# NicolaDM/MAPLE

Measured on AMD Instinct MI355X. Metric: candidate SPR placements/sec, higher is better.
Workload: dtype f64

## Files before the change

include/maple_hip_debug.h:

```cpp
#ifndef MAPLE_HIP_DEBUG_H
#define MAPLE_HIP_DEBUG_H
#include "maple_hip.h"

#ifdef __cplusplus
extern "C" {
#endif

int maple_debug_frontier_levels(maple_ctx *ctx, int32_t cap, int64_t *itemsUpdating, int64_t *itemsCached, float *msUpdating,
                                float *msCached, int32_t *n, int64_t *waveItemsSmall , int64_t *waveItemsBig );

int maple_debug_wave_append_batch(maple_ctx *ctx, int32_t n, const int32_t *parentList, const int32_t *childList,
                                  const uint8_t *isTipC, const double *bLen, double *outLK, float *ms);
int maple_debug_trace_query(maple_ctx *ctx, int32_t query);
int maple_debug_calib_walk(maple_ctx *ctx, uint64_t bytes, int32_t repeats, float *ms);
int maple_debug_calib_write(maple_ctx *ctx, uint64_t bytes, int32_t mode, int32_t repeats, float *ms);
int maple_debug_trace_read(maple_ctx *ctx, int32_t *n, int32_t *items4 , double *vals2 );
int maple_debug_gpv_batch(maple_ctx *ctx, int32_t n, const int32_t *i12, const double *totLen, const double *M16,
                          const double *errorRate, const double *vect4, const uint8_t *upNode, const uint8_t *flag,
                          double *out4);
int maple_debug_simplify_batch(maple_ctx *ctx, int32_t n, const double *vec4, const int32_t *refA, int32_t *out);
int maple_debug_frontier_pass_batch(maple_ctx *ctx, int32_t n, const int32_t *list, const int32_t *mutList, const uint8_t *dirIsUp,
                                    int32_t waveForm, int32_t *outList, uint8_t *grade, uint8_t *sameHandle);

#ifdef __cplusplus
}
#endif
#endif
```

maple_amd/csrc/batch_host.h:

```cpp
#pragma once
#include "ctx_host.h"

#include <algorithm>
#include <cstring>
#include <vector>

struct alignas(16) TileBest { double score; int32_t rank, idx; };

#ifndef MAPLE_BLOCK
#define MAPLE_BLOCK 256
#endif
#ifndef MAPLE_APPEND_WAVES
#define MAPLE_APPEND_WAVES 4
#endif
#define MAPLE_APPEND_ATTR __launch_bounds__(MAPLE_BLOCK) __attribute__((amdgpu_waves_per_eu(MAPLE_APPEND_WAVES, MAPLE_APPEND_WAVES)))
#ifndef MAPLE_ZERO_DIST_BUDGET
#define MAPLE_ZERO_DIST_BUDGET 16
#endif

static int grid_for(int n)
{
    int g = (n + MAPLE_BLOCK - 1) / MAPLE_BLOCK;
    if (g < 1) g = 1;
    if (g > 256 * 8) g = 256 * 8;
// ... 13 lines not shown
static inline int ev_pair(maple_ctx *c, hipEvent_t *a, hipEvent_t *b, int kind = 0, double units = 0.0, double bytes = 0.0)
{
    return maple_internal_ev_pair(c, a, b, kind, units, bytes);
}

template <class T> static int h2d(maple_ctx *c, DevBuf<T> &b, const T *src, size_t n)
{
    HIPCK(c, b.reserve(n ? n : 1));
    if (n) HIPCK(c, hipMemcpyAsync(b.p, src, n * sizeof(T), hipMemcpyHostToDevice, c->stream));
    return MAPLE_OK;
}

static int stage_begin(maple_ctx *c, size_t bytes)
{
    c->stg_cur ^= 1;
    const int k = c->stg_cur;
    bytes += 4096;
    if (bytes > c->stg_cap[k]) {
        HIPCK(c, hipStreamSynchronize(c->stream));
        if (c->stg_h[k]) (void)hipHostFree(c->stg_h[k]);
        if (c->stg_d[k]) (void)hipFree(c->stg_d[k]);
        c->stg_h[k] = nullptr; c->stg_d[k] = nullptr; c->stg_cap[k] = 0;
        const size_t want = std::max(bytes * 2, (size_t)1 << 20);
        HIPCK(c, hipHostMalloc((void **)&c->stg_h[k], want, hipHostMallocDefault));
        HIPCK(c, hipMalloc((void **)&c->stg_d[k], want));
        c->stg_cap[k] = want;
    }
    c->stg_used = c->stg_flushed = 0;
    return MAPLE_OK;
}
template <class T> static T *stage_put(maple_ctx *c, const T *src, size_t n)
{
    const int k = c->stg_cur;
    const size_t off = (c->stg_used + 15) & ~(size_t)15, bytes = n * sizeof(T);
    if (off + bytes > c->stg_cap[k]) return nullptr;
    if (bytes) memcpy(c->stg_h[k] + off, src, bytes);
    c->stg_used = off + bytes;
    return (T *)(c->stg_d[k] + off);
}
static int stage_flush(maple_ctx *c)
{
    const int k = c->stg_cur;
    if (c->stg_used > c->stg_flushed)
        HIPCK(c, hipMemcpyAsync(c->stg_d[k] + c->stg_flushed, c->stg_h[k] + c->stg_flushed, c->stg_used - c->stg_flushed,
                                hipMemcpyHostToDevice, c->stream));
    c->stg_flushed = c->stg_used;
    return MAPLE_OK;
}
#define STAGE(var, c, src, n) auto *var = stage_put((c), (src), (size_t)(n)); if (!var) return fail((c), MAPLE_ERR_NOMEM, "argument staging overflow")

static int need_model(maple_ctx *c)
{
    if (!c->model_set) return fail(c, MAPLE_ERR_STATE, "maple_set_model has not been called");
    return MAPLE_OK;
}


__attribute__((visibility("hidden")))
int commit_lists(maple_ctx *c, int32_t n, const int64_t *d_woff, const int64_t *d_aoff, int32_t *d_n_ent, int32_t *d_n_aux,
                 int32_t *outList, const uint2 *srcW = nullptr, const double *srcA = nullptr);
__attribute__((visibility("hidden")))
int commit_known(maple_ctx *c, int32_t n, const int64_t *d_woff, const int64_t *d_aoff, const int32_t *d_n_ent, const int32_t *d_n_aux,
                 const std::vector<int32_t> &ne, const std::vector<int32_t> &na, int32_t *outList, const uint2 *srcW, const double *srcA);
__attribute__((visibility("hidden")))
int settle(maple_ctx *c);
__attribute__((visibility("hidden")))
int evaluate_placement_items(maple_ctx *c, int32_t n, const int32_t *midTot, const int32_t *down, const int32_t *up, const double *dist,
                             const int32_t *rem, const uint8_t *remTip, const uint8_t *fromTip1, double *out4, double *comp2);
__attribute__((visibility("hidden")))
void launch_wave_append(maple_ctx *c, int grid, int n, const int32_t *pl, const int32_t *cl, const uint8_t *tip, const double *bl, double *out);
__attribute__((visibility("hidden")))
int launch_append_queries(maple_ctx *c, hipStream_t s, int nQ, const int32_t *qList, int nC, const int32_t *cand, int isTip, double bLen,
                          double *out, long long ldOut, const int32_t *outCol, const uint8_t *qTip, const double *qBLen, int kind,
                          double algBytes, TileBest *tileBest = nullptr, const int32_t *visitRank = nullptr, const int4 *chunkTab = nullptr,
                          int nChunkTab = 0, int nF = 1, unsigned long long *finMask = nullptr, bool lanesOnly = false);
__attribute__((visibility("hidden")))
int launch_place_score(maple_ctx *c, int nQ, int nF, const int32_t *qFrameLists, int nC, const int32_t *cand, const int32_t *candFrame,
                       int isTip, double bLen, double *out, long long ldOut, const int32_t *outCol, const uint8_t *qTip, const double *qBLen,
                       int kind = MAPLE_K_PLACE_SCORE, double algBytes = 0.0);
__attribute__((visibility("hidden")))
void update_scratch_free(maple_ctx *c);
__attribute__((visibility("hidden")))
int tree_rebuild_from_host(maple_ctx *c);
```

maple_amd/csrc/debug_abi.hip:

```cpp
#include "../../include/maple_hip_debug.h"
#include "genome_dev.h"
#include "ctx_host.h"
#include "batch_host.h"
#include "frontier.h"
#include "frontier_dev.h"

#include <algorithm>

using namespace frt;

__global__ __launch_bounds__(MAPLE_BLOCK) void k_calib_walk(const unsigned long long *buf, long long nLists, unsigned long long *sink)
{
    unsigned long long acc = 0;
    for (long long l = (long long)blockIdx.x * blockDim.x + threadIdx.x; l < nLists; l += (long long)gridDim.x * blockDim.x) {
        const unsigned long long *p = buf + l * 64;
        unsigned idx = 0;
        for (int k = 0; k < 64; k++) {
            unsigned long long w = p[idx];
            acc += w;
            idx = (idx + 1 + (unsigned)(w & 0)) & 63;
        }
    }
    if (acc == 0x123456789abcdefull) *sink = acc;
}
// ... 210 lines not shown
                                                              int32_t *nAux, uint8_t *grade)
{
    for (int i = blockIdx.x * blockDim.x + threadIdx.x; i < n; i += gridDim.x * blockDim.x) {
        const int h = handle[i];
        if (h >= 0 && h < fp.capL) {
            const LRec r = fp.trec[h];
            woff[i] = LREC_OFF(r.x); aoff[i] = LREC_OFF(r.y); nEnt[i] = LREC_N(r.x); nAux[i] = LREC_N(r.y); grade[i] = fp.tflag[h];
        } else { woff[i] = 0; aoff[i] = 0; nEnt[i] = -1; nAux[i] = 0; grade[i] = 0; }
    }
}

extern "C" int maple_debug_frontier_pass_batch(maple_ctx *c, int32_t n, const int32_t *list, const int32_t *mutList, const uint8_t *dirIsUp,
                                               int32_t waveForm, int32_t *outList, uint8_t *grade, uint8_t *sameHandle)
{
    if (!c || n < 0 || n > (1 << 20) || !list || !mutList || !dirIsUp || !outList || !grade || !sameHandle) return MAPLE_ERR_ARG;
    if (n == 0) return MAPLE_OK;
    HIPCK(c, hipSetDevice(c->device));
    TRY(need_model(c));
    TRY(check_ids(c, n, list, false, "list"));
    TRY(settle(c));
    const int32_t nml = (int32_t)c->h_mut_cnt.size();
    long long capW = 0, capA = 0;
    int capE = 1;
    for (int i = 0; i < n; i++) {
        if (mutList[i] < -1 || mutList[i] >= nml) return fail(c, MAPLE_ERR_ARG, "mutList[%d] = %d is not a mutation-list id", i, mutList[i]);
        const long long cnt = mutList[i] < 0 ? 0 : c->h_mut_cnt[mutList[i]];
        const long long ne = c->h_n_ent[list[i]] + 2 * cnt, na = c->h_n_aux[list[i]] + 4 * cnt;
        capW += ne; capA += na;
        capE = std::max(capE, (int)ne);
    }
    const int threads = waveForm ? 64 * std::min(n, 1024) : std::min(1024, (n + FR_BLOCK - 1) / FR_BLOCK * FR_BLOCK);
    const int grid = (threads + FR_BLOCK - 1) / FR_BLOCK;
    const long long lanes = (long long)grid * FR_BLOCK;
    HIPCK(c, c->s_words.reserve((size_t)capW));
    HIPCK(c, c->s_aux.reserve((size_t)capA));
    auto up16 = [](size_t x) { return (x + 255) & ~(size_t)255; };
    const size_t oRec = 0, oCtr = up16(oRec + (size_t)n * sizeof(LRec)), oSw = up16(oCtr + sizeof(FCtr)),
                 oSa = up16(oSw + (waveForm ? 0 : (size_t)lanes * capE * sizeof(uint2))),
                 oWoff = up16(oSa + (waveForm ? 0 : (size_t)lanes * 5 * capE * sizeof(double))), oAoff = up16(oWoff + (size_t)n * 8),
                 oHandle = up16(oAoff + (size_t)n * 8), oNe = up16(oHandle + (size_t)n * 4), oNa = up16(oNe + (size_t)n * 4),
                 oFlag = up16(oNa + (size_t)n * 4), oGrade = up16(oFlag + (size_t)n), total = up16(oGrade + (size_t)n);
    uint8_t *buf = nullptr;
    HIPCK(c, hipMalloc((void **)&buf, total));
    int rc = MAPLE_OK;
    std::vector<int32_t> handle(n);
    do {
        if (hipMemsetAsync(buf, 0, oSw, c->stream) != hipSuccess) { rc = fail(c, MAPLE_ERR_HIP, "hipMemsetAsync"); break; }
        FPools fp;
        memset(&fp, 0, sizeof fp);
        fp.tw = c->s_words.p; fp.ta = c->s_aux.p;
        fp.trec = (LRec *)(buf + oRec); fp.tflag = buf + oFlag;
        fp.capW = capW; fp.capA = capA; fp.capL = n;
        fp.sw = (uint2 *)(buf + oSw); fp.sa = (double *)(buf + oSa); fp.capE = capE;
        fp.ctr = (FCtr *)(buf + oCtr);
        fp.mat = 1;
        fp.mv = MutViewS{c->d_mut3, c->d_mut_off, c->d_mut_cnt};
        const ArenaViewS av{c->d_words, c->d_aux, c->d_ent_off, c->d_aux_off, c->d_n_ent, c->d_n_aux};
        if ((rc = stage_begin(c, (size_t)n * 64 + 256)) != MAPLE_OK) break;
        auto *dl = stage_put(c, list, (size_t)n);
        auto *dml = stage_put(c, mutList, (size_t)n);
        auto *dup = stage_put(c, dirIsUp, (size_t)n);
        if (!dl || !dml || !dup) { rc = fail(c, MAPLE_ERR_NOMEM, "argument staging overflow"); break; }
        if ((rc = stage_flush(c)) != MAPLE_OK) break;
        int32_t *dHandle = (int32_t *)(buf + oHandle), *dNe = (int32_t *)(buf + oNe), *dNa = (int32_t *)(buf + oNa);
        int64_t *dWoff = (int64_t *)(buf + oWoff), *dAoff = (int64_t *)(buf + oAoff);
        if (waveForm) DISPATCH3(c, k_debug_fpass_wave, <<<grid, FR_BLOCK, 0, c->stream>>>(c->d_model, av, fp, n, dl, dml, dup, dHandle));
        else DISPATCH3(c, k_debug_fpass_lane, <<<grid, FR_BLOCK, 0, c->stream>>>(c->d_model, av, fp, n, dl, dml, dup, dHandle));
        hipLaunchKernelGGL(k_debug_fpass_out, dim3(grid_for(n)), dim3(FR_BLOCK), 0, c->stream, fp, n, dHandle, dWoff, dAoff, dNe, dNa, buf + oGrade);
        if (hipGetLastError() != hipSuccess || hipMemcpyAsync(handle.data(), dHandle, (size_t)n * 4, hipMemcpyDeviceToHost, c->stream) != hipSuccess
            || hipMemcpyAsync(grade, buf + oGrade, (size_t)n, hipMemcpyDeviceToHost, c->stream) != hipSuccess
            || hipStreamSynchronize(c->stream) != hipSuccess) { rc = fail(c, MAPLE_ERR_HIP, "the frontier pass hook's launch failed"); break; }
        for (int i = 0; i < n && rc == MAPLE_OK; i++) {
            sameHandle[i] = handle[i] == -(list[i] + 10);
            if (!sameHandle[i] && handle[i] < 0) rc = fail(c, MAPLE_ERR_NOMEM, "item %d: no room for the new list (%d)", i, handle[i]);
        }
        if (rc != MAPLE_OK) break;
        if ((rc = commit_lists(c, n, dWoff, dAoff, dNe, dNa, outList, fp.tw, fp.ta)) != MAPLE_OK) break;
        if (hipStreamSynchronize(c->stream) != hipSuccess) { rc = fail(c, MAPLE_ERR_HIP, "hipStreamSynchronize"); break; }
        for (int i = 0; i < n; i++) if (sameHandle[i]) outList[i] = list[i];
    } while (0);
    (void)hipFree(buf);
    return rc;
}
```

maple_amd/csrc/spr_batch.hip:

```cpp
#include "../../include/maple_hip.h"
#include "genome_dev.h"
#include "search_dev.h"
#include "placement_dev.h"
#include "append_lds.h"
#include "wave_dev.h"
#include "wave_update.h"

#include <algorithm>
#include <chrono>
#include <cfloat>
#include <cmath>
#include <cstdarg>
#include <cstdio>
#include <cstring>
#include <functional>
#include <string>
#include <vector>

using namespace maple;

#include <hipcub/hipcub.hpp>
#include "ctx_host.h"
#include "batch_host.h"
#include "frontier.h"
// ... 837 lines not shown

    const int32_t nT = c->dtree.n;
    std::vector<int32_t> byRank(nT, -1);
    for (int i = 0; i < nT; i++) byRank[c->h_nodes[i].preRank] = i;
    std::vector<SScan> sc((size_t)nT);
    std::vector<int32_t> size(nT, 1), depth(nT, 0);
    std::vector<uint8_t> reach(nT, 0);
    int32_t maxDepth = 0;
    if (!c->tree_stale && c->place && (int)c->h_depth.size() == nT && !c->place->order.empty() && c->place->order[0] == c->dtree.root) {
        for (const int32_t v : c->place->order) { reach[v] = 1; depth[v] = c->h_depth[v]; maxDepth = std::max(maxDepth, depth[v]); }
    } else {
        std::vector<int32_t> stk{c->dtree.root};
        while (!stk.empty()) {
            const int v = stk.back();
            stk.pop_back();
            reach[v] = 1;
            if (c->h_tree_c0[v] >= 0) { stk.push_back(c->h_tree_c0[v]); stk.push_back(c->h_tree_c1[v]); }
        }
        for (int r = 0; r < nT; r++) {
            const int v = byRank[r];
            const int u = c->h_tree_up[v];
            if (reach[v] && u >= 0 && v != c->dtree.root && c->h_nodes[u].preRank < r) depth[v] = depth[u] + 1;
            maxDepth = std::max(maxDepth, depth[v]);
        }
    }
    for (int r = nT - 1; r >= 0; r--) {
        const int v = byRank[r];
        const int u = c->h_tree_up[v];
        if (reach[v] && u >= 0 && v != c->dtree.root && c->h_nodes[u].preRank < r) size[u] += size[v];
    }
    for (int r = 0; r < nT; r++) {
        const int v = byRank[r];
        const NodeRec &nr = c->h_nodes[v];
        uint32_t fl = 0;
        if (nr.up >= 0 && (nr.dist > P.effNon0 || nr.upIsRoot)) fl |= SS_SCORED;
        if (nr.totUp >= 0) fl |= SS_TOTUP;
        if (nr.c0 >= 0) fl |= SS_INNER;
        if (nr.up >= 0 && (nr.whichChild ? c->h_nodes[nr.up].upLeft : c->h_nodes[nr.up].upRight) >= 0) fl |= SS_ENTER;
        sc[r] = SScan{v, size[v], depth[v], ((uint32_t)nr.frameOf << 4) | fl};
    }
    std::vector<int32_t> prank((size_t)nT, 0);
    for (int r = 0; r < nT; r++) { const int u = c->h_tree_up[byRank[r]]; prank[r] = u >= 0 ? c->h_nodes[u].preRank : 0; }
    std::vector<int32_t> candBefore((size_t)nT + 1, 0), cladeVisits((size_t)nT, 0);
    for (int r = 0; r < nT; r++)
        candBefore[r + 1] = candBefore[r] + ((sc[r].ff & SS_TOTUP) ? 1 : 0);
    for (int r = nT - 1; r >= 1; r--) {
        const int v = byRank[r];
        if (!reach[v]) continue;
        const uint32_t fl = sc[r].ff & 15u;
        if (!(fl & SS_ENTER)) continue;
        const bool scored = fl & SS_SCORED, counts = scored && (fl & SS_TOTUP), dropped = scored && !(fl & SS_TOTUP);
        const int add = (counts ? 1 : 0) + ((!dropped && (fl & SS_INNER)) ? cladeVisits[r] : 0);
        cladeVisits[prank[r]] += add;
    }
    TRY(h2d(c, c->t_cand_before, candBefore.data(), candBefore.size()));
    TRY(h2d(c, c->t_clade_visits, cladeVisits.data(), cladeVisits.size()));
    TRY(h2d(c, c->t_scan, sc.data(), sc.size()));
    TRY(h2d(c, c->t_scan_parent, prank.data(), prank.size()));
    HIPCK(c, hipStreamSynchronize(c->stream));
    c->tree_max_depth = maxDepth;
    c->scan_eff = P.effNon0;
    c->scan_valid = true;
    return MAPLE_OK;
}

__global__ __launch_bounds__(64) void k_finite_prefix(int nRows, int nWords, const unsigned long long *mask, int32_t *prefix)
{
    const int lane = threadIdx.x;
    for (int row = blockIdx.x; row < nRows; row += gridDim.x) {
        const unsigned long long *m = mask + (size_t)row * nWords;
        int32_t *p = prefix + (size_t)row * (nWords + 1);
        int run = 0;
        for (int base = 0; base <= nWords; base += 64) {
            const int w = base + lane;
            const int cnt = w < nWords ? __popcll(m[w]) : 0;
            int incl = cnt;
            for (int off = 1; off < 64; off <<= 1) { const int t = __shfl_up(incl, off, 64); if (lane >= off) incl += t; }
            if (w <= nWords) p[w] = run + incl - cnt;
            run += __shfl(incl, 63, 64);
        }
    }
}

static int lists_to_root_frame(maple_ctx *c, std::vector<int32_t> &ids, std::vector<int32_t> fr)
{
    const PlaceMeta &Fm = *c->place;
    std::vector<int32_t> who, src, ml, out;
    std::vector<uint8_t> dir;
    for (;;) {
        who.clear(); src.clear(); ml.clear();
        for (size_t k = 0; k < ids.size(); k++)
            if (fr[k] != 0 && ids[k] >= 0) { who.push_back((int32_t)k); src.push_back(ids[k]); ml.push_back(c->h_tree_mut[Fm.frameNode[fr[k]]]); }
        if (who.empty()) return MAPLE_OK;
        dir.assign(who.size(), 1);
        out.resize(who.size());
        TRY(maple_pass_branch_batch(c, (int32_t)who.size(), src.data(), ml.data(), dir.data(), out.data()));
        for (size_t i = 0; i < who.size(); i++) { ids[who[i]] = out[i]; fr[who[i]] = Fm.frameParent[fr[who[i]]]; }
    }
}
static int ensure_cand_root(maple_ctx *c)
{
    if (c->cand_root_end >= 0) return MAPLE_OK;
    if (c->cand_root_mark >= 0 && c->cand_root_top == (int64_t)c->h_n_ent.size())
        TRY(maple_arena_release(c, c->cand_root_mark | ((int64_t)c->h_mut_cnt.size() << 40)));
    c->cand_root_mark = c->cand_root_top = -1;
    const int64_t begin = (int64_t)c->h_n_ent.size();
    std::vector<int32_t> candRoot(c->h_cand_ids);
    TRY(lists_to_root_frame(c, candRoot, c->h_cand_frame));
    TRY(h2d(c, c->s_cand_root, candRoot.data(), candRoot.size()));
    HIPCK(c, hipStreamSynchronize(c->stream));
    c->cand_root_end = (int64_t)c->h_n_ent.size();
    c->cand_root_mark = begin; c->cand_root_top = c->cand_root_end;
    return MAPLE_OK;
}

extern "C" int maple_spr_search_batch(maple_ctx *c, int32_t n, const int32_t *nodes, const maple_search_params *sp,
                                      int32_t ws_entries_per_lane, int32_t *bestNode, double *bestScore, double *blen3,
                                      int32_t *placement, double *improvement, double *currentLK, int32_t *nAppend,
                                      int32_t *status, int32_t *outRprList)
{
    if (!c || n < 0 || !nodes || !sp || !bestNode || !bestScore || !blen3 || !placement || !improvement || !currentLK
        || !nAppend || !status)
        return MAPLE_ERR_ARG;
    if (n == 0) return MAPLE_OK;
    HIPCK(c, hipSetDevice(c->device));
    TRY(need_model(c));
    if (!c->tree_set) return fail(c, MAPLE_ERR_STATE, "maple_tree_upload has not been called");
    for (int i = 0; i < n; i++)
        if (nodes[i] < 0 || nodes[i] >= c->dtree.n) return fail(c, MAPLE_ERR_ARG, "nodes[%d] = %d is not a node", i, nodes[i]);
    bool patchedOnly = false;
    c->last_search_frontier_only = false;
    if (c->tree_stale) {
        patchedOnly = c->nodes_current && !c->tree_has_mut && n <= 64 && sp->searchTier == 0 && c->trace_query < 0 && !outRprList;
        for (int i = 0; i < n && patchedOnly; i++)
            if (sp->wideSearchBudget >= 0 && !c->dm.usingErrorRate && c->h_tree_dist[nodes[i]] == 0.0) patchedOnly = false;
        if (!patchedOnly) TRY(tree_rebuild_from_host(c));
    }
    const bool dbgT = c->tuning.verbose != 0;
    auto tnow = [] { return std::chrono::steady_clock::now(); };
    auto tms = [](std::chrono::steady_clock::time_point a, std::chrono::steady_clock::time_point b) {
        return std::chrono::duration_cast<std::chrono::microseconds>(b - a).count() * 1e-3;
    };
    const auto tStart = tnow();
    SearchParams P;
    P.strict = sp->strictTopologyStopRules; P.allowedFails = sp->allowedFailsTopology;
    P.thrLKtopology = sp->thresholdLogLKtopology; P.thrPlacement = sp->thresholdTopologyPlacement;
    P.thrOptTopo = sp->thresholdLogLKoptimizationTopology; P.thrConsec = sp->thresholdLogLKconsecutivePlacement;
    P.effNon0 = sp->effectivelyNon0BLen;
    HIPCK(c, c->s_search_out.reserve((size_t)n * sizeof(SearchOut)));
    HIPCK(c, c->s_counter.reserve(8));
    std::vector<SearchOut> &ho = c->h_search_out;
    ho.assign((size_t)n, SearchOut{});
    std::vector<uint8_t> hintedNow;
    std::vector<int32_t> todo(nodes, nodes + n), slot(n);
    for (int i = 0; i < n; i++) slot[i] = i;
    long long poolCapW = 0, poolCapA = 0;
    uint2 *poolW = nullptr;
    double *poolA = nullptr;
    if (outRprList) {
        for (int i = 0; i < n; i++) {
            int lid = c->h_tree_lower[nodes[i]];
            long long ne = lid >= 0 ? c->h_n_ent[lid] : 0, na = lid >= 0 ? c->h_n_aux[lid] : 0;
            poolCapW += 3 * ne + 64; poolCapA += 3 * na + 5 * ne + 64;
        }
        HIPCK(c, c->s_pool_w.reserve((size_t)poolCapW));
        HIPCK(c, c->s_pool_a.reserve((size_t)poolCapA));
        poolW = c->s_pool_w.p; poolA = c->s_pool_a.p;
    }
    HIPCK(c, hipMemsetAsync(c->s_counter.p, 0, 8 * sizeof(int32_t), c->stream));
    unsigned long long *poolUsed = (unsigned long long *)(c->s_counter.p + 2);
    if (dbgT) fprintf(stderr, "[maple] t=%.1f ms: result records cleared\n", tms(tStart, tnow()));
    const int capW0 = ws_entries_per_lane > 0 ? ws_entries_per_lane : std::max(16384, 64 * c->tree_max_ent);
    bool heavyQueries = false;
    bool assistOK = !c->dm.usingErrorRate;
    const bool assistFew = !c->dm.usingErrorRate;
    const bool useFrontier = sp->searchTier == 0 && c->trace_query < 0;
    const std::vector<int32_t> *rowOverride = nullptr;
    FiniteRows finRows{nullptr, nullptr, 0};
    const int finWords = (c->n_scored + 63) / 64;
    auto fin_reserve = [&](size_t rows) -> int {
        HIPCK(c, c->s_fin_mask.reserve_exact(std::max(rows * (size_t)finWords, c->s_fin_mask.cap)));
        HIPCK(c, c->s_fin_prefix.reserve_exact(std::max(rows * (size_t)(finWords + 1), c->s_fin_prefix.cap)));
// ... 175 lines not shown
    std::vector<int32_t> preIdx, preRowOf;
    int preSpare = 0;
    const int nTpre = c->dtree.n;
    const bool matPre = c->tree_has_mut;
    int64_t preMark = -1;
    std::vector<int32_t> preFrameParent, preFrameNode;
    auto pre_rows_max = [&]() -> size_t {
        size_t freeB = 0, totalB = 0;
        size_t budgetB = (size_t)4ull << 30;
        if (hipMemGetInfo(&freeB, &totalB) == hipSuccess)
            budgetB = std::max(budgetB, std::min((freeB + c->s_cache.cap * sizeof(double)) / 2, (size_t)96ull << 30));
        return budgetB / ((size_t)nTpre * sizeof(double));
    };
    auto pre_rows = [&](const bool witnessOK) -> int {
        const size_t rowsMax = pre_rows_max();
        if (preIdx.size() < 64 || preIdx.size() > rowsMax) preIdx.clear();
        else {
            preSpare = witnessOK ? (int)std::min<size_t>(4096, rowsMax - preIdx.size()) : 0;
            const int mZ = (int)preIdx.size();
            HIPCK(c, c->s_cache.reserve_exact((size_t)(mZ + preSpare) * nTpre));
            TRY(fin_reserve((size_t)mZ + preSpare));
            if (!c->stream2) {
                HIPCK(c, hipStreamCreateWithFlags(&c->stream2, hipStreamNonBlocking));
                HIPCK(c, hipEventCreateWithFlags(&c->ev_fork, hipEventDisableTiming));
                HIPCK(c, hipEventCreateWithFlags(&c->ev_join, hipEventDisableTiming));
            }
            std::vector<int32_t> ql(mZ);
            std::vector<uint8_t> qt(mZ);
            std::vector<double> qb(mZ);
            preRowOf.assign(n, -1);
            double qBytes = 0.0;
            for (int k = 0; k < mZ; k++) {
                const int node = nodes[preIdx[k]];
                ql[k] = c->h_tree_lower[node]; qt[k] = c->h_tree_tip[node]; qb[k] = c->h_tree_dist[node];
                preRowOf[preIdx[k]] = k;
                qBytes += 8.0 * c->h_n_ent[ql[k]] + 8.0 * c->h_n_aux[ql[k]];
                if (witnessOK && qb[k] != 0.0) return fail(c, MAPLE_ERR_FATAL, "a search with removedBLen %g among the searches of the witness filter", qb[k]);
            }
            if (matPre) {
                const PlaceMeta &Fm = *c->place;
                TRY(ensure_cand_root(c));
                TRY(maple_arena_mark(c, &preMark));
                std::vector<int32_t> qf(mZ);
                for (int k = 0; k < mZ; k++) qf[k] = Fm.frameOf[nodes[preIdx[k]]];
                TRY(lists_to_root_frame(c, ql, qf));
                if (dbgT) fprintf(stderr, "[maple] t=%.1f ms: their removed lists in the root's frame\n", tms(tStart, tnow()));
                preFrameParent = Fm.frameParent;
                preFrameNode = Fm.frameNode;
                useFin = true;
            }
            HIPCK(c, c->z_ql.reserve(mZ)); HIPCK(c, c->z_qt.reserve(mZ)); HIPCK(c, c->z_qb.reserve(mZ));
            HIPCK(c, hipEventRecord(c->ev_fork, c->stream));
            HIPCK(c, hipStreamWaitEvent(c->stream2, c->ev_fork, 0));
            HIPCK(c, hipMemcpyAsync(c->z_ql.p, ql.data(), (size_t)mZ * sizeof(int32_t), hipMemcpyHostToDevice, c->stream2));
            HIPCK(c, hipMemcpyAsync(c->z_qt.p, qt.data(), (size_t)mZ, hipMemcpyHostToDevice, c->stream2));
            HIPCK(c, hipMemcpyAsync(c->z_qb.p, qb.data(), (size_t)mZ * sizeof(double), hipMemcpyHostToDevice, c->stream2));
            HIPCK(c, hipStreamSynchronize(c->stream2));
            afterLaunch = [c, mZ, nTpre, qBytes, fin_prefix, useFin, finWords, dbgT, matPre, witnessOK]() -> int {
                if (witnessOK && useFin && !c->tuning.denseWideScoring) {
                    long long pairs = 0;
                    TRY(witness_score(c, c->stream2, mZ, c->z_ql.p, c->z_qt.p, c->z_qb.p, c->n_scored, matPre ? c->s_cand_root.p : c->t_i32[8].p,
                                      matPre ? c->t_cand_rank.p : c->t_scored_col.p,
                                      c->s_cache.p, nTpre, c->s_fin_mask.p, finWords,
                                      c->n_scored ? c->scored_bytes_total / c->n_scored : 0.0, qBytes, &pairs));
                    if (dbgT) fprintf(stderr, "[maple] witness filter: %lld of %lld (search, branch) pairs walked\n", pairs, (long long)mZ * c->n_scored);
                    TRY(fin_prefix(c->stream2, 0, (size_t)mZ));
                    HIPCK(c, hipEventRecord(c->ev_join, c->stream2));
                    return MAPLE_OK;
                }
                TRY(launch_append_queries(c, c->stream2, mZ, c->z_ql.p, c->n_scored, matPre ? c->s_cand_root.p : c->t_i32[8].p, 0, 0.0, c->s_cache.p, nTpre,
                                          matPre ? c->t_cand_rank.p : c->t_scored_col.p, c->z_qt.p, c->z_qb.p, MAPLE_K_SPR_SCORE,
                                          (double)mZ * c->scored_bytes_total + qBytes, nullptr, nullptr, nullptr, 0, 1, useFin ? c->s_fin_mask.p : nullptr));
                if (useFin) TRY(fin_prefix(c->stream2, 0, (size_t)mZ));
                HIPCK(c, hipEventRecord(c->ev_join, c->stream2));
                return MAPLE_OK;
            };
            if (dbgT) fprintf(stderr, "[maple] t=%.1f ms: %d searches %s to be scored on the side stream\n", tms(tStart, tnow()), mZ,
                              witnessOK ? "from zero-length branches" : "that ran over the budget the last time");
        }
        return MAPLE_OK;
    };
    if (hybrid && !c->dm.usingErrorRate && wideBudget > 16 && (!matPre || (c->scan_valid && c->place && !c->tuning.noCladeScan && !c->tuning.denseWideScoring && !c->tuning.wideOutsideFrontier))) {
        {
            std::vector<int32_t> zi, pl, cl;
            std::vector<uint8_t> tp;
            for (int i = 0; i < n; i++) {
                const int v = nodes[i], u = c->h_tree_up[v];
                if (c->h_tree_dist[v] != 0.0 || u < 0) continue;
                if (matPre && c->h_tree_mut[v] >= 0) continue;
                const int32_t vu = c->h_tree_c0[u] == v ? c->h_tree_upRight[u] : c->h_tree_upLeft[u];
                if (vu < 0 || c->h_tree_lower[v] < 0) continue;
                zi.push_back(i); pl.push_back(vu); cl.push_back(c->h_tree_lower[v]); tp.push_back(c->h_tree_tip[v]);
            }
            if (zi.size() >= 64) {
                std::vector<double> bl(zi.size(), 0.0), cur(zi.size());
                const int rc = maple_append_batch(c, (int32_t)zi.size(), pl.data(), cl.data(), tp.data(), bl.data(), cur.data());
                if (rc != MAPLE_OK) return rc;
                for (size_t k = 0; k < zi.size(); k++) if (cur[k] < P.thrPlacement) preIdx.push_back(zi[k]);
            }
            if (dbgT) fprintf(stderr, "[maple] t=%.1f ms: current placements of %zu nodes on zero-length branches scored\n", tms(tStart, tnow()), zi.size());
        }
        TRY(pre_rows(true));
    } else if (hybrid && c->dm.usingErrorRate && useFrontier && !c->tuning.noOverHint && (int)c->h_over_hint.size() >= c->dtree.n && wideBudget > 16
               && c->scan_valid && c->place && !c->tuning.noCladeScan && !c->tuning.wideOutsideFrontier) {
        const size_t rowsMax = pre_rows_max();
        for (int i = 0; i < n && preIdx.size() < rowsMax; i++)
            if (c->h_over_hint[nodes[i]] && !(matPre && c->h_tree_mut[nodes[i]] >= 0)) preIdx.push_back(i);
        TRY(pre_rows(false));
    }
    if (useFrontier) {
        if (dbgT) fprintf(stderr, "[maple] t=%.1f ms: prologue done\n", tms(tStart, tnow()));
        if (afterLaunch) { std::function<int()> f; f.swap(afterLaunch); TRY(f()); }
        if (dbgT) fprintf(stderr, "[maple] t=%.1f ms: side-stream scoring queued\n", tms(tStart, tnow()));
        FrontierStats fs;
        const int frontierBudget = !hybrid ? 0 : (c->dm.usingErrorRate ? wideBudget
                                                                       : std::max(wideBudget, sp->wideSearchBudget == 0 ? c->n_scored / 2 : 0));
        FrontierWide fw{nullptr, nullptr, FiniteRows{nullptr, nullptr, 0}, nullptr, 0};
        if (!preIdx.empty() && !c->tuning.wideOutsideFrontier) {
            fw.rowOf = preRowOf.data(); fw.cacheS = c->s_cache.p; fw.rowsReady = c->ev_join;
            if (useFin) fw.fin = FiniteRows{c->s_fin_mask.p, c->s_fin_prefix.p, finWords};
            if (matPre) {
                TRY(h2d(c, c->s_frame_parent, preFrameParent.data(), preFrameParent.size()));
                TRY(h2d(c, c->s_frame_node, preFrameNode.data(), preFrameNode.size()));
                fw.frameParent = c->s_frame_parent.p; fw.frameNode = c->s_frame_node.p; fw.nFrames = (int)preFrameParent.size();
            }
        }
        std::vector<uint8_t> overHint;
        if (hybrid && c->dm.usingErrorRate && !c->tuning.noOverHint && (int)c->h_over_hint.size() >= c->dtree.n) {
            overHint.resize((size_t)n);
            size_t nHint = 0;
            hintedNow.assign((size_t)n, 0);
            for (int i = 0; i < n; i++) {
                hintedNow[i] = c->h_over_hint[todo[i]];
                overHint[i] = hintedNow[i] && !(!preRowOf.empty() && preRowOf[i] >= 0);
                nHint += overHint[i];
            }
            if (!nHint) overHint.clear();
            else if (dbgT) fprintf(stderr, "[maple] t=%.1f ms: %zu searches that ran over the budget last time go to the dense tier at once\n", tms(tStart, tnow()), nHint);
        }
        TRY(frontier_search(c, P, n, todo.data(), frontierBudget, (hybrid && wideBudget > MAPLE_ZERO_DIST_BUDGET) ? MAPLE_ZERO_DIST_BUDGET : (1 << 30),
                            ho.data(), poolW, poolA, poolUsed, poolCapW, poolCapA, &fs, 0, fw.rowOf ? &fw : nullptr,
                            overHint.empty() ? nullptr : overHint.data()));
        if (hybrid && c->dm.usingErrorRate) {
            if ((int)c->h_over_hint.size() < c->dtree.n) c->h_over_hint.resize((size_t)c->dtree.n, 0);
            for (int i = 0; i < n; i++)
                if (ho[i].status == -5 && ho[i].nAppend >= 0 && (overHint.empty() || !overHint[i])) c->h_over_hint[todo[i]] = 1;
        }
        std::vector<int32_t> todoFb, slotFb;
        for (int i = 0; i < n; i++)
            if (ho[i].status == FR_STATUS_FALLBACK) { todoFb.push_back(todo[i]); slotFb.push_back(i); }
        if (dbgT)
            fprintf(stderr, "[maple] t=%.1f ms: frontier tier done: %d levels, %lld updating + %lld cached items, %lld temporary lists "
                            "(%lld words, %lld aux), %lld refined records, %zu searches handed back%s\n", tms(tStart, tnow()), fs.levels,
                    fs.itemsUpdating, fs.itemsCached, fs.tempLists, fs.tempWords, fs.tempAux, fs.records, todoFb.size(),
                    fs.overflow ? " (a pool overflowed)" : "");
        c->last_search_frontier_only = todoFb.empty() && !hybrid;
        if (!todoFb.empty()) TRY(run_queries(todoFb, slotFb, nullptr, hybrid ? wideBudget : 0, nullptr, 0));
    } else
        TRY(run_queries(todo, slot, nullptr, hybrid ? wideBudget : 0, nullptr, 0));
    if (dbgT) fprintf(stderr, "[maple] t=%.1f ms: budgeted pass done\n", tms(tStart, tnow()));
    if (hybrid) {
        std::vector<int32_t> wide;
        for (int i = 0; i < n; i++)
            if (ho[i].status == -5) { wide.push_back(i); if (ho[i].bestNode == -2) heavyQueries = true; }
        if (!preIdx.empty()) {
            const int mZ = (int)preIdx.size();
            std::vector<int32_t> qn, sl, rowsNow, rest, ql2;
            std::vector<uint8_t> qt2;
            std::vector<double> qb2;
            for (int32_t i : wide) {
                const int node = nodes[i];
                if (matPre) { rest.push_back(i); continue; }
                if (preRowOf[i] >= 0) { qn.push_back(node); sl.push_back(i); rowsNow.push_back(preRowOf[i]); }
                else if ((int)ql2.size() < preSpare) {
                    qn.push_back(node); sl.push_back(i); rowsNow.push_back(mZ + (int)ql2.size());
                    ql2.push_back(c->h_tree_lower[node]); qt2.push_back(c->h_tree_tip[node]); qb2.push_back(c->h_tree_dist[node]);
                } else rest.push_back(i);
            }
            if (!ql2.empty()) {
                const int m2 = (int)ql2.size();
                TRY(h2d(c, c->s_i32[6], ql2.data(), (size_t)m2));
                TRY(h2d(c, c->s_u8[3], qt2.data(), (size_t)m2));
                TRY(h2d(c, c->s_f64[3], qb2.data(), (size_t)m2));
// ... 288 lines not shown
```

maple_amd/runtime.py:

```python
from __future__ import annotations

import ctypes as C
import os

import numpy as np

from .genome_list import PackedLists, pack_lists, pack_mutations, unpack_list

HERE = os.path.dirname(os.path.abspath(__file__))
LIB_PATH = os.path.join(HERE, "libmaple_hip.so")

EXPORTS = [
    "maple_abi_version", "maple_create", "maple_destroy", "maple_set_tuning", "maple_last_error", "maple_set_model", "maple_get_model",
    "maple_lists_upload", "maple_lists_update", "maple_lists_sizes", "maple_lists_download", "maple_arena_mark", "maple_arena_release",
    "maple_arena_stats", "maple_mutations_upload", "maple_append_batch", "maple_merge_batch", "maple_blen_batch",
    "maple_differ_batch", "maple_pass_branch_batch", "maple_shorten_batch", "maple_root_vector_batch",
    "maple_evaluate_placement_batch", "maple_update_partials", "maple_update_partials_touched", "maple_tree_patch", "maple_append_batch_dev", "maple_append_queries_dev", "maple_timing_reset", "maple_timing_read", "maple_timing_read_each",
    "maple_append_algorithmic_bytes", "maple_tree_upload", "maple_spr_search_batch", "maple_minor_batch", "maple_root_prob_batch", "maple_candset_create", "maple_append_candset",
    "maple_minor_candset", "maple_placement_search_batch", "maple_placement_prepare", "maple_placement_ahead", "maple_placement_ahead_stats", "maple_set_fatal_policy",
    "maple_timing_read_kind", "maple_placement_supports_batch",
    "maple_candset_destroy", "maple_spr_search_visited", "maple_arena_compact", "maple_append_queries_argmax_dev", "maple_comm_unique_id", "maple_comm_init", "maple_argmax_allreduce_dev", "maple_tree_rebuild_lists",
]


DEBUG_EXPORTS = ["maple_debug_wave_append_batch", "maple_debug_trace_query", "maple_debug_trace_read", "maple_debug_calib_walk",
                 "maple_debug_calib_write", "maple_debug_gpv_batch", "maple_debug_simplify_batch", "maple_debug_frontier_levels",
                 "maple_debug_frontier_pass_batch"]
LIB_PATH_DEBUG = os.path.join(HERE, "libmaple_hip_debug.so")


class MapleParams(C.Structure):
    _fields_ = [("thresholdProb", C.c_double), ("minBLenSensitivity", C.c_double),
                ("thresholdDiffForUpdate", C.c_double), ("thresholdFoldChangeUpdate", C.c_double),
                ("defaultBLen", C.c_double)]


class MapleSearchParams(C.Structure):
    _fields_ = [("strictTopologyStopRules", C.c_int32), ("allowedFailsTopology", C.c_int32),
                ("thresholdLogLKtopology", C.c_double), ("thresholdTopologyPlacement", C.c_double),
                ("thresholdLogLKoptimizationTopology", C.c_double), ("thresholdLogLKconsecutivePlacement", C.c_double),
                ("effectivelyNon0BLen", C.c_double), ("wideSearchBudget", C.c_int32), ("searchTier", C.c_int32)]


class MapleTuning(C.Structure):
    _fields_ = [("structSize", C.c_uint32), ("wavePerItemMax", C.c_int32), ("placementChunkMax", C.c_int32), ("noCladeScan", C.c_int32), ("verbose", C.c_int32),
                ("wideOutsideFrontier", C.c_int32), ("denseWideScoring", C.c_int32), ("waveAllBelow", C.c_int32), ("noOverHint", C.c_int32), ("noAheadExpansion", C.c_int32), ("noAheadSpeculation", C.c_int32)]


class MaplePlacementParams(C.Structure):
    _fields_ = [("oneMutBLen", C.c_double), ("effectivelyNon0BLen", C.c_double), ("thresholdLogLK", C.c_double),
                ("thresholdLogLKoptimization", C.c_double), ("thresholdLogLKconsecutivePlacement", C.c_double),
                ("allowedFails", C.c_int32), ("strictStopRules", C.c_int32), ("onlyFindIdentical", C.c_int32)]


class MapleError(RuntimeError):
    ERR_ARG, ERR_HIP, ERR_NOMEM, ERR_STATE, ERR_FATAL = -1, -2, -3, -4, -5

    def __init__(self, msg, code=None):
        super().__init__(msg)
        self.code = code


_lib = None
_lib_debug = None


def load_library(debug=False):
    global _lib, _lib_debug
    if (_lib_debug if debug else _lib) is None:
        default = LIB_PATH_DEBUG if debug else LIB_PATH
        lib_path = os.environ.get("MAPLE_HIP_LIB_DEBUG" if debug else "MAPLE_HIP_LIB", default)
        if not os.path.exists(lib_path):
            raise MapleError(f"{lib_path} is missing: run `python -c 'import __graft_entry__ as g; g.build()'`; "
                             "there is no CPU fallback for the placement path")
        try:
            import torch
        except ImportError:
            pass
        lib = C.CDLL(lib_path)
        lib.maple_last_error.restype = C.c_char_p
        for name in EXPORTS + (DEBUG_EXPORTS if debug else []):
            if not hasattr(lib, name):
                raise MapleError(f"{lib_path} does not export {name} (include/maple_hip{'_debug' if name in DEBUG_EXPORTS else ''}.h): "
                                 "rebuild it with __graft_entry__.build()")
        if debug:
            _lib_debug = lib
        else:
            _lib = lib
    return _lib_debug if debug else _lib


def _ptr(a):
    return None if a is None else a.ctypes.data_as(C.c_void_p)


def _i32(x):
    return np.ascontiguousarray(x, dtype=np.int32)


def _u8(x):
    return np.ascontiguousarray(x, dtype=np.uint8)


def _f64(x):
    return np.ascontiguousarray(x, dtype=np.float64)


class Device:

    def __init__(self, ref_idx, root_freqs, *, device=0, thresholdProb=1e-8, minBLenSensitivity=None,
# ... 330 lines not shown
                                  thresholdLogLKconsecutivePlacement, int(allowedFails), int(bool(strictStopRules)),
                                  int(bool(onlyFindIdentical)))
        self._ck(self.lib.maple_placement_prepare(self.h, C.byref(pp)))

    def placement_ahead(self, q_lists, *, oneMutBLen, effectivelyNon0BLen, thresholdLogLK, thresholdLogLKoptimization,
                        thresholdLogLKconsecutivePlacement, allowedFails=5, strictStopRules=True, onlyFindIdentical=False):
        q = _i32(q_lists)
        pp = MaplePlacementParams(oneMutBLen, effectivelyNon0BLen, thresholdLogLK, thresholdLogLKoptimization,
                                  thresholdLogLKconsecutivePlacement, int(allowedFails), int(bool(strictStopRules)),
                                  int(bool(onlyFindIdentical)))
        taken = C.c_int32(0)
        self._ck(self.lib.maple_placement_ahead(self.h, len(q), _ptr(q), C.byref(pp), C.byref(taken)))
        return taken.value

    def placement_ahead_stats(self):
        out = np.zeros(5, dtype=np.int64)
        self._ck(self.lib.maple_placement_ahead_stats(self.h, _ptr(out)))
        return dict(zip(("searches", "fallbacks", "expanded_items", "traversals_ahead_used", "traversals_ahead_dropped"), (int(x) for x in out)))

    def placement_search_batch(self, q_lists, *, oneMutBLen, effectivelyNon0BLen, thresholdLogLK,
                               thresholdLogLKoptimization, thresholdLogLKconsecutivePlacement, allowedFails=5,
                               strictStopRules=True, onlyFindIdentical=False):
        q = _i32(q_lists)
        n = len(q)
        pp = MaplePlacementParams(oneMutBLen, effectivelyNon0BLen, thresholdLogLK, thresholdLogLKoptimization,
                                  thresholdLogLKconsecutivePlacement, int(allowedFails), int(bool(strictStopRules)),
                                  int(bool(onlyFindIdentical)))
        out = dict(bestNode=np.zeros(n, np.int32), bestScore=np.zeros(n), blen=np.zeros((n, 3)),
                   bestDiffs=np.zeros(n, np.int32), nAppend=np.zeros(n, np.int32), status=np.zeros(n, np.int32))
        self._ck(self.lib.maple_placement_search_batch(self.h, n, _ptr(q), C.byref(pp), _ptr(out["bestNode"]),
                                                       _ptr(out["bestScore"]), _ptr(out["blen"]), _ptr(out["bestDiffs"]),
                                                       _ptr(out["nAppend"]), _ptr(out["status"])))
        return out

    def placement_supports_batch(self, q_lists, *, oneMutBLen, effectivelyNon0BLen, thresholdLogLK,
                                 thresholdLogLKoptimization, thresholdLogLKconsecutivePlacement,
                                 thresholdLogLKoptimizationTopology, minBranchSupport=0.01, allowedFails=5,
                                 strictStopRules=True, onlyFindIdentical=False):
        q = _i32(q_lists)
        n = len(q)
        pp = MaplePlacementParams(oneMutBLen, effectivelyNon0BLen, thresholdLogLK, thresholdLogLKoptimization,
                                  thresholdLogLKconsecutivePlacement, int(allowedFails), int(bool(strictStopRules)),
                                  int(bool(onlyFindIdentical)))
        cap = 128 * max(1, n)
        off = np.zeros(n + 1, np.int64)
        node, supp, bl = np.zeros(cap, np.int32), np.zeros(cap), np.zeros((cap, 3))
        best, status = np.zeros(n, np.int32), np.zeros(n, np.int32)
        self._ck(self.lib.maple_placement_supports_batch(self.h, n, _ptr(q), C.byref(pp),
                                                         C.c_double(thresholdLogLKoptimizationTopology),
                                                         C.c_double(minBranchSupport), C.c_int64(cap), _ptr(off), _ptr(node),
                                                         _ptr(supp), _ptr(bl), _ptr(best), _ptr(status)))
        out = []
        for g in range(n):
            a, b = off[g], off[g + 1]
            out.append(([(int(node[i]), float(supp[i]), tuple(float(x) for x in bl[i])) for i in range(a, b)], int(best[g])))
        return out, status

    def debug_gpv_batch(self, i12, totLen, mutMatrix, errorRate, vect, upNode, flag):
        i12 = _i32(i12)
        n = len(i12)
        M = _f64(np.asarray(mutMatrix, dtype=np.float64).reshape(n, 16))
        v = _f64(np.asarray(vect, dtype=np.float64).reshape(n, 4))
        out = np.zeros((n, 4))
        self._ck(self.lib.maple_debug_gpv_batch(self.h, n, _ptr(i12), _ptr(_f64(totLen)), _ptr(M), _ptr(_f64(errorRate)), _ptr(v),
                                                _ptr(_u8(upNode)), _ptr(_u8(flag)), _ptr(out)))
        return out

    def debug_simplify_batch(self, vec, refA):
        v = _f64(np.asarray(vec, dtype=np.float64).reshape(-1, 4))
        out = np.zeros(len(v), dtype=np.int32)
        self._ck(self.lib.maple_debug_simplify_batch(self.h, len(v), _ptr(v), _ptr(_i32(refA)), _ptr(out)))
        return out

    def debug_frontier_pass_batch(self, lists, mutLists, dirIsUp, wave_form=False):
        lists, mutLists = _i32(lists), _i32(mutLists)
        n = len(lists)
        up = _u8(np.broadcast_to(dirIsUp, n))
        out = np.zeros(n, dtype=np.int32)
        grade, same = np.zeros(n, dtype=np.uint8), np.zeros(n, dtype=np.uint8)
        self._ck(self.lib.maple_debug_frontier_pass_batch(self.h, n, _ptr(lists), _ptr(mutLists), _ptr(up), int(bool(wave_form)),
                                                          _ptr(out), _ptr(grade), _ptr(same)))
        return out, grade, same.astype(bool)

    def debug_calib_walk(self, nbytes, repeats=1):
        ms = C.c_float()
        self._ck(self.lib.maple_debug_calib_walk(self.h, C.c_uint64(nbytes), int(repeats), C.byref(ms)))
        return ms.value

    def debug_calib_write(self, nbytes, mode, repeats=1):
        ms = C.c_float()
        self._ck(self.lib.maple_debug_calib_write(self.h, C.c_uint64(nbytes), int(mode), int(repeats), C.byref(ms)))
        return ms.value

    def debug_trace_query(self, q):
        self._ck(self.lib.maple_debug_trace_query(self.h, int(q)))

    def debug_trace_read(self):
        n = C.c_int32()
        it = np.zeros(4 * 4096, dtype=np.int32)
        va = np.zeros(2 * 4096, dtype=np.float64)
        self._ck(self.lib.maple_debug_trace_read(self.h, C.byref(n), _ptr(it), _ptr(va)))
        k = min(n.value, 4096)
        return it[: 4 * k].reshape(k, 4), va[: 2 * k].reshape(k, 2)

    def append_batch_dev(self, n, parent_ptr, child_ptr, tip_ptr, blen_ptr, out_ptr, stream=0):
        self._ck(self.lib.maple_append_batch_dev(self.h, int(n), C.c_void_p(parent_ptr), C.c_void_p(child_ptr),
                                                 C.c_void_p(tip_ptr), C.c_void_p(blen_ptr), C.c_void_p(out_ptr),
                                                 C.c_void_p(stream)))

    def append_queries_dev(self, nQ, qlist_ptr, nC, cand_ptr, isTipC, bLen, out_ptr, stream=0):
        self._ck(self.lib.maple_append_queries_dev(self.h, int(nQ), C.c_void_p(qlist_ptr), int(nC), C.c_void_p(cand_ptr),
                                                   int(bool(isTipC)), C.c_double(bLen), C.c_void_p(out_ptr),
                                                   C.c_void_p(stream)))

    def append_queries_argmax_dev(self, nQ, qlist_ptr, nC, cand_ptr, rank_ptr, isTipC, bLen, best_score_ptr, best_idx_ptr, stream=0):
        self._ck(self.lib.maple_append_queries_argmax_dev(self.h, int(nQ), C.c_void_p(qlist_ptr), int(nC), C.c_void_p(cand_ptr),
                                                          C.c_void_p(rank_ptr), int(bool(isTipC)), C.c_double(bLen),
                                                          C.c_void_p(best_score_ptr), C.c_void_p(best_idx_ptr), C.c_void_p(stream)))

    def comm_unique_id(self):
        buf = np.zeros(128, dtype=np.uint8)
        self._ck(self.lib.maple_comm_unique_id(self.h, _ptr(buf)))
        return buf

    def comm_init(self, world, rank, unique_id):
        self._ck(self.lib.maple_comm_init(self.h, int(world), int(rank), _ptr(_u8(unique_id))))

    def argmax_allreduce_dev(self, n, score_ptr, idx_ptr, stream=0):
        self._ck(self.lib.maple_argmax_allreduce_dev(self.h, int(n), C.c_void_p(score_ptr), C.c_void_p(idx_ptr), C.c_void_p(stream)))

    def timing_reset(self):
        self._ck(self.lib.maple_timing_reset(self.h))

    def timing_read_each(self, cap=256):
        ms = np.zeros(cap, dtype=np.float32)
        n = C.c_int32()
        self._ck(self.lib.maple_timing_read_each(self.h, int(cap), _ptr(ms), C.byref(n)))
        return ms[: n.value].tolist()

    def frontier_levels(self, cap=4096):
        iu, ic = np.zeros(cap, np.int64), np.zeros(cap, np.int64)
        ws, wb = np.zeros(cap, np.int64), np.zeros(cap, np.int64)
        mu, mc = np.zeros(cap, np.float32), np.zeros(cap, np.float32)
        n = C.c_int32()
        self._ck(self.lib.maple_debug_frontier_levels(self.h, int(cap), _ptr(iu), _ptr(ic), _ptr(mu), _ptr(mc), C.byref(n), _ptr(ws), _ptr(wb)))
        k = min(cap, n.value)
        self.last_wave_items = (ws[:k], wb[:k])
        return iu[:k], ic[:k], mu[:k], mc[:k]

    def tree_rebuild_lists(self, root, up, c0, c1, tip, mut, dist, lower, bump_len=0.0):
        n = len(up)
        up, c0, c1 = _i32(up), _i32(c0), _i32(c1)
        tip = np.ascontiguousarray(np.asarray(tip, np.uint8))
        mutp = None if mut is None else _i32(mut)
        assert dist.dtype == np.float64 and dist.flags.c_contiguous
        lower = _i32(lower).copy()
        ur, ul, tu = (np.full(n, -1, np.int32) for _ in range(3))
        bad = np.zeros(max(64, n), np.int32)
        nbad = C.c_int32()
        self._ck(self.lib.maple_tree_rebuild_lists(self.h, n, int(root), _ptr(up), _ptr(c0), _ptr(c1), _ptr(tip), _ptr(mutp), _ptr(dist),
                                                   _ptr(lower), _ptr(ur), _ptr(ul), _ptr(tu), C.c_double(bump_len), len(bad), _ptr(bad),
                                                   C.byref(nbad)))
        return lower, ur, ul, tu, np.unique(bad[: min(nbad.value, len(bad))])

    def timing_read(self):
        n, ms = C.c_int32(), C.c_double()
# ... 19 lines not shown
```

Baseline: 42.61 billion.

## Fuse frame-chain passes into one kernel and score zero-length placements on device

lists_to_root_frame used to issue one host-driven pass_branch batch per frame level, looping until every item reached the root frame. It now runs the whole frame chain for each item in a single kernel, ping-ponging between two scratch halves, and commits all results once, with chunking to bound scratch size. The current-placement scoring of nodes on zero-length branches is also moved from host-gathered append_batch calls into a device kernel that reads the tree directly and returns flags. The aim is fewer launches, host round trips and syncs, at the cost of large scratch reservations and per-thread serial chains. A debug export is added for testing.

```diff
diff --git a/include/maple_hip_debug.h b/include/maple_hip_debug.h
--- a/include/maple_hip_debug.h
+++ b/include/maple_hip_debug.h
@@ -21,6 +21,7 @@
 int maple_debug_simplify_batch(maple_ctx *ctx, int32_t n, const double *vec4, const int32_t *refA, int32_t *out);
 int maple_debug_frontier_pass_batch(maple_ctx *ctx, int32_t n, const int32_t *list, const int32_t *mutList, const uint8_t *dirIsUp,
                                     int32_t waveForm, int32_t *outList, uint8_t *grade, uint8_t *sameHandle);
+int maple_debug_lists_to_root_frame(maple_ctx *ctx, int32_t n, const int32_t *list, const int32_t *node, int32_t *outList);
 
 #ifdef __cplusplus
 }
diff --git a/maple_amd/csrc/batch_host.h b/maple_amd/csrc/batch_host.h
--- a/maple_amd/csrc/batch_host.h
+++ b/maple_amd/csrc/batch_host.h
@@ -119,3 +119,5 @@
 void update_scratch_free(maple_ctx *c);
 __attribute__((visibility("hidden")))
 int tree_rebuild_from_host(maple_ctx *c);
+__attribute__((visibility("hidden")))
+int lists_to_root_frame(maple_ctx *c, std::vector<int32_t> &ids, const std::vector<int32_t> &fr);
diff --git a/maple_amd/csrc/debug_abi.hip b/maple_amd/csrc/debug_abi.hip
--- a/maple_amd/csrc/debug_abi.hip
+++ b/maple_amd/csrc/debug_abi.hip
@@ -316,3 +316,21 @@
     (void)hipFree(buf);
     return rc;
 }
+
+extern "C" int maple_debug_lists_to_root_frame(maple_ctx *c, int32_t n, const int32_t *list, const int32_t *node, int32_t *outList)
+{
+    if (!c || n < 0 || (n && (!list || !node || !outList))) return MAPLE_ERR_ARG;
+    if (n == 0) return MAPLE_OK;
+    HIPCK(c, hipSetDevice(c->device));
+    if (!c->tree_set || !c->place) return fail(c, MAPLE_ERR_STATE, "maple_tree_upload has not been called");
+    TRY(check_ids(c, n, list, true, "list"));
+    std::vector<int32_t> ids(list, list + n), fr(n, 0);
+    for (int i = 0; i < n; i++) {
+        if (node[i] >= c->dtree.n) return fail(c, MAPLE_ERR_ARG, "node[%d] = %d is not a node", i, node[i]);
+        fr[i] = node[i] < 0 ? 0 : c->place->frameOf[node[i]];
+    }
+    TRY(lists_to_root_frame(c, ids, fr));
+    HIPCK(c, hipStreamSynchronize(c->stream));
+    memcpy(outList, ids.data(), (size_t)n * sizeof(int32_t));
+    return MAPLE_OK;
+}
diff --git a/maple_amd/csrc/spr_batch.hip b/maple_amd/csrc/spr_batch.hip
--- a/maple_amd/csrc/spr_batch.hip
+++ b/maple_amd/csrc/spr_batch.hip
@@ -943,22 +943,100 @@
     }
 }
 
-static int lists_to_root_frame(maple_ctx *c, std::vector<int32_t> &ids, std::vector<int32_t> fr)
+__global__ __launch_bounds__(MAPLE_BLOCK) void k_pass_chain(int lRef, ArenaView av, MutView mv, int n, const int32_t *l, const int32_t *fr,
+                                                            const int32_t *frameParent, const int32_t *frameMut, uint2 *words, double *aux,
+                                                            const int64_t *woff, const int64_t *aoff, int64_t *fwoff, int64_t *faoff,
+                                                            int32_t *n_ent, int32_t *n_aux)
+{
+    for (int i = blockIdx.x * blockDim.x + threadIdx.x; i < n; i += gridDim.x * blockDim.x) {
+        const int64_t w0 = woff[i], sw = (woff[i + 1] - w0) >> 1, a0 = aoff[i], sa = (aoff[i + 1] - a0) >> 1;
+        ListRef cur = list_ref(av, l[i]);
+        int side = 0, r = 0, na = 0;
+        for (int f = fr[i]; f > 0; f = frameParent[f]) {
+            Writer w;
+            w.init(words + w0 + side * sw, aux + a0 + side * sa);
+            const int id = frameMut[f];
+            r = pass_walk(lRef, cur, mv.mut3 + 3 * mv.off[id], mv.cnt[id], true, w);
+            na = w.na;
+            cur = ListRef{w.w, w.aux};
+            side ^= 1;
+        }
+        fwoff[i] = cur.w - words; faoff[i] = cur.aux - aux;
+        n_ent[i] = r; n_aux[i] = na;
+    }
+}
+
+#ifndef MAPLE_CHAIN_SCRATCH_ENTRIES
+#define MAPLE_CHAIN_SCRATCH_ENTRIES ((int64_t)1 << 26)
+#endif
+int lists_to_root_frame(maple_ctx *c, std::vector<int32_t> &ids, const std::vector<int32_t> &fr)
 {
     const PlaceMeta &Fm = *c->place;
-    std::vector<int32_t> who, src, ml, out;
-    std::vector<uint8_t> dir;
-    for (;;) {
-        who.clear(); src.clear(); ml.clear();
-        for (size_t k = 0; k < ids.size(); k++)
-            if (fr[k] != 0 && ids[k] >= 0) { who.push_back((int32_t)k); src.push_back(ids[k]); ml.push_back(c->h_tree_mut[Fm.frameNode[fr[k]]]); }
-        if (who.empty()) return MAPLE_OK;
-        dir.assign(who.size(), 1);
-        out.resize(who.size());
-        TRY(maple_pass_branch_batch(c, (int32_t)who.size(), src.data(), ml.data(), dir.data(), out.data()));
-        for (size_t i = 0; i < who.size(); i++) { ids[who[i]] = out[i]; fr[who[i]] = Fm.frameParent[fr[who[i]]]; }
-    }
-}
+    const int nF = (int)Fm.frameNode.size();
+    if (nF <= 1 || ids.empty()) return MAPLE_OK;
+    std::vector<int32_t> who, src, sfr, fmut(nF, -1), out;
+    std::vector<int64_t> chainMut(nF, 0);
+    for (int f = 1; f < nF; f++) {
+        fmut[f] = c->h_tree_mut[Fm.frameNode[f]];
+        chainMut[f] = chainMut[Fm.frameParent[f]] + c->h_mut_cnt[fmut[f]];
+    }
+    for (size_t k = 0; k < ids.size(); k++) {
+        if (fr[k] == 0 || ids[k] < 0) continue;
+        if (fr[k] < 0 || fr[k] >= nF) return fail(c, MAPLE_ERR_ARG, "frame %d of item %zu is not a frame of the tree (%d)", fr[k], k, nF);
+        who.push_back((int32_t)k); src.push_back(ids[k]); sfr.push_back(fr[k]);
+    }
+    if (who.empty()) return MAPLE_OK;
+    TRY(check_ids(c, (int32_t)src.size(), src.data(), false, "list"));
+    std::vector<int64_t> woff, aoff;
+    for (size_t b = 0; b < who.size();) {
+        woff.assign(1, 0); aoff.assign(1, 0);
+        size_t e = b;
+        while (e < who.size()) {
+            const int64_t sw = (int64_t)c->h_n_ent[src[e]] + 2 * chainMut[sfr[e]], sa = (int64_t)c->h_n_aux[src[e]] + 4 * chainMut[sfr[e]];
+            if (e > b && woff.back() + 2 * sw > MAPLE_CHAIN_SCRATCH_ENTRIES) break;
+            woff.push_back(woff.back() + 2 * sw); aoff.push_back(aoff.back() + 2 * sa);
+            e++;
+        }
+        const int m = (int)(e - b);
+        HIPCK(c, c->s_words.reserve((size_t)woff.back()));
+        HIPCK(c, c->s_aux.reserve((size_t)std::max<int64_t>(aoff.back(), 1)));
+        TRY(stage_begin(c, (size_t)m * 48 + (size_t)nF * 8 + 512));
+        STAGE(dl, c, src.data() + b, m); STAGE(dfr, c, sfr.data() + b, m); STAGE(dwo, c, woff.data(), m + 1); STAGE(dao, c, aoff.data(), m + 1);
+        STAGE(dfp, c, Fm.frameParent.data(), nF); STAGE(dfm, c, fmut.data(), nF);
+        TRY(stage_flush(c));
+        HIPCK(c, c->s_i32[2].reserve(m)); HIPCK(c, c->s_i32[3].reserve(m));
+        HIPCK(c, c->s_i64[4].reserve(m)); HIPCK(c, c->s_i64[5].reserve(m));
+        hipLaunchKernelGGL(k_pass_chain, dim3(grid_for(m)), dim3(MAPLE_BLOCK), 0, c->stream, c->lRef, view(c), mview(c), m, dl, dfr, dfp, dfm,
+                           c->s_words.p, c->s_aux.p, dwo, dao, c->s_i64[4].p, c->s_i64[5].p, c->s_i32[2].p, c->s_i32[3].p);
+        HIPCK(c, hipGetLastError());
+        out.resize(m);
+        TRY(commit_lists(c, m, c->s_i64[4].p, c->s_i64[5].p, c->s_i32[2].p, c->s_i32[3].p, out.data()));
+        for (int i = 0; i < m; i++) ids[who[b + i]] = out[i];
+        b = e;
+    }
+    return MAPLE_OK;
+}
+template <bool RV, bool U, bool SS>
+__global__ MAPLE_APPEND_ATTR void k_cur_placement(const DevModel *__restrict__ mp, ArenaView av, DevTree T, int n, const int32_t *nodes,
+                                                  int hasMut, double thr, uint8_t *flag)
+{
+    __shared__ Lds lds;
+    const DevModel &m = *mp;
+    stage_model(m, lds);
+    Ctx<RV, U, SS> c(m, lds);
+    for (int i = blockIdx.x * blockDim.x + threadIdx.x; i < n; i += gridDim.x * blockDim.x) {
+        const int v = nodes[i];
+        const NodeRec &r = T.nd[v];
+        uint8_t f = 0;
+        if (r.dist == 0.0 && r.up >= 0 && !(hasMut && r.mutId >= 0) && r.lower >= 0) {
+            const NodeRec &p = T.nd[r.up];
+            const int32_t vu = p.c0 == v ? p.upRight : p.upLeft;
+            if (vu >= 0) f = append_walk(c, list_ref(av, vu), list_ref(av, r.lower), r.isTip != 0, 0.0) < thr ? 2 : 1;
+        }
+        flag[i] = f;
+    }
+}
+
 static int ensure_cand_root(maple_ctx *c)
 {
     if (c->cand_root_end >= 0) return MAPLE_OK;
@@ -1300,23 +1378,24 @@
     };
     if (hybrid && !c->dm.usingErrorRate && wideBudget > 16 && (!matPre || (c->scan_valid && c->place && !c->tuning.noCladeScan && !c->tuning.denseWideScoring && !c->tuning.wideOutsideFrontier))) {
         {
-            std::vector<int32_t> zi, pl, cl;
-            std::vector<uint8_t> tp;
-            for (int i = 0; i < n; i++) {
-                const int v = nodes[i], u = c->h_tree_up[v];
-                if (c->h_tree_dist[v] != 0.0 || u < 0) continue;
-                if (matPre && c->h_tree_mut[v] >= 0) continue;
-                const int32_t vu = c->h_tree_c0[u] == v ? c->h_tree_upRight[u] : c->h_tree_upLeft[u];
-                if (vu < 0 || c->h_tree_lower[v] < 0) continue;
-                zi.push_back(i); pl.push_back(vu); cl.push_back(c->h_tree_lower[v]); tp.push_back(c->h_tree_tip[v]);
-            }
-            if (zi.size() >= 64) {
-                std::vector<double> bl(zi.size(), 0.0), cur(zi.size());
-                const int rc = maple_append_batch(c, (int32_t)zi.size(), pl.data(), cl.data(), tp.data(), bl.data(), cur.data());
-                if (rc != MAPLE_OK) return rc;
-                for (size_t k = 0; k < zi.size(); k++) if (cur[k] < P.thrPlacement) preIdx.push_back(zi[k]);
-            }
-            if (dbgT) fprintf(stderr, "[maple] t=%.1f ms: current placements of %zu nodes on zero-length branches scored\n", tms(tStart, tnow()), zi.size());
+            size_t nZero = 0;
+            if (n >= 64) {
+                TRY(stage_begin(c, (size_t)n * 4 + 256));
+                STAGE(dnodes, c, nodes, n);
+                TRY(stage_flush(c));
+                HIPCK(c, c->s_u8[0].reserve((size_t)n));
+                HIPCK(c, c->pin_res.reserve((size_t)n));
+                DISPATCH3(c, k_cur_placement, <<<grid_for(n), MAPLE_BLOCK, 0, c->stream>>>(c->d_model, view(c), c->dtree, n, dnodes, matPre ? 1 : 0,
+                                                                                          P.thrPlacement, c->s_u8[0].p));
+                HIPCK(c, hipGetLastError());
+                const uint8_t *hf = (const uint8_t *)c->pin_res.p;
+                HIPCK(c, hipMemcpyAsync(c->pin_res.p, c->s_u8[0].p, (size_t)n, hipMemcpyDeviceToHost, c->stream));
+                HIPCK(c, hipStreamSynchronize(c->stream));
+                for (int i = 0; i < n; i++) nZero += hf[i] != 0;
+                if (nZero >= 64)
+                    for (int i = 0; i < n; i++) if (hf[i] == 2) preIdx.push_back(i);
+            }
+            if (dbgT) fprintf(stderr, "[maple] t=%.1f ms: current placements of %zu nodes on zero-length branches scored\n", tms(tStart, tnow()), nZero);
         }
         TRY(pre_rows(true));
     } else if (hybrid && c->dm.usingErrorRate && useFrontier && !c->tuning.noOverHint && (int)c->h_over_hint.size() >= c->dtree.n && wideBudget > 16
diff --git a/maple_amd/runtime.py b/maple_amd/runtime.py
--- a/maple_amd/runtime.py
+++ b/maple_amd/runtime.py
@@ -25,7 +25,7 @@
 
 DEBUG_EXPORTS = ["maple_debug_wave_append_batch", "maple_debug_trace_query", "maple_debug_trace_read", "maple_debug_calib_walk",
                  "maple_debug_calib_write", "maple_debug_gpv_batch", "maple_debug_simplify_batch", "maple_debug_frontier_levels",
-                 "maple_debug_frontier_pass_batch"]
+                 "maple_debug_frontier_pass_batch", "maple_debug_lists_to_root_frame"]
 LIB_PATH_DEBUG = os.path.join(HERE, "libmaple_hip_debug.so")
 
 
@@ -522,6 +522,12 @@
                                                           _ptr(out), _ptr(grade), _ptr(same)))
         return out, grade, same.astype(bool)
 
+    def debug_lists_to_root_frame(self, lists, nodes):
+        lists, nodes = _i32(lists), _i32(nodes)
+        out = np.zeros(len(lists), dtype=np.int32)
+        self._ck(self.lib.maple_debug_lists_to_root_frame(self.h, len(lists), _ptr(lists), _ptr(nodes), _ptr(out)))
+        return out
+
     def debug_calib_walk(self, nbytes, repeats=1):
         ms = C.c_float()
         self._ck(self.lib.maple_debug_calib_walk(self.h, C.c_uint64(nbytes), int(repeats), C.byref(ms)))
```

Result: faster. 44.26 billion, median of 6 (+3.9%).
